# wenxuanliu/multimodal-vae

Measured on AMD Instinct MI355X. Metric: ELBO-steps/sec (whole node), MultiMNIST b=256 per GPU, higher is better.
Workload: dtype bf16; 1 GPU; multimnist_50x50_conv_mmvae_gru_text_3pass_elbo_step; batch_per_gpu=256, global_batch=256, n_latents=100, parallelism=dp1, hip_graph=False, optimizer=adam, mfma=bf16 in / fp32 acc; fp32 master weights, BN stats, PoE/KL/BCE/NLL, Adam

## Files before the change

### multimodal-vae_amd/csrc/gemm_small.hip

```cpp
#include "gemm.h"
#include <cstdlib>

namespace {

typedef __attribute__((ext_vector_type(4))) int i32x4;

__device__ __forceinline__ bf16x8 buf_load16(__amdgpu_buffer_rsrc_t rsrc, unsigned off) {
    const i32x4 v = __builtin_bit_cast(i32x4, __builtin_amdgcn_raw_buffer_load_b128(rsrc, (int)off, 0, 0));
    return __builtin_bit_cast(bf16x8, v);
}

__device__ __forceinline__ int fast_divmod(int r, int d, float inv, int& rem) {
    int q = (int)((float)r * inv);
    rem = r - q * d;
    if (rem < 0) { --q; rem += d; }
    else if (rem >= d) { ++q; rem -= d; }
    return q;
}

template <int MT, int NT, int KS, bool DGRAD>
__global__ __launch_bounds__(KS * 64) void gemm_small_kernel(const GemmParams p) {
    extern __shared__ __attribute__((aligned(16))) char smem[];
    const GatherCommon& c = p.c;
    const GatherClass& k = p.cls[blockIdx.z];
    const int tid = threadIdx.x, lane = tid & 63, wave = tid >> 6;
    const int fr = lane & 15, fq = lane >> 4;
    constexpr int RW = MT * 16, CW = NT * 16;
    const int tiles_per_group = (k.rows_per_group + RW - 1) / RW;
    if ((int)blockIdx.x >= tiles_per_group * c.groups) return;
    const int g = blockIdx.x / tiles_per_group;
    const int row0 = (blockIdx.x - g * tiles_per_group) * RW;
    const int n_base = blockIdx.y * CW;
    const int K = k.K, Kpad = k.Kpad;
    const int nch_all = (K + 63) / 64;
    const int ch0 = nch_all * wave / KS, ch1 = nch_all * (wave + 1) / KS;

    const int nimg_a = c.a_bcast_n > 0 ? c.a_bcast_n : c.groups * c.group_n;
    const __amdgpu_buffer_rsrc_t arsrc = __builtin_amdgcn_make_buffer_rsrc(
        const_cast<bf16*>(c.A), 0, (int)((size_t)nimg_a * c.AH * c.AW * c.Ald * sizeof(bf16)), 0x00020000);
    const __amdgpu_buffer_rsrc_t brsrc = __builtin_amdgcn_make_buffer_rsrc(
        const_cast<bf16*>(k.Wp), 0, (int)((size_t)p.npad * Kpad * sizeof(bf16)), 0x00020000);

    const int pix_per_img = k.OY * k.OX;
    const float inv_pix = 1.0f / (float)pix_per_img, inv_ox = 1.0f / (float)k.OX, inv_tw = 1.0f / (float)k.TW;
    int a_off[MT], opix[MT], dpix[MT], grow[MT];
    unsigned mtap[MT];
#pragma unroll
    for (int mt = 0; mt < MT; ++mt) {
        const int r = row0 + mt * 16 + fr;
        a_off[mt] = 0; mtap[mt] = 0; opix[mt] = -1; dpix[mt] = 0; grow[mt] = 0;
        if (r < k.rows_per_group) {
            int rem, ox;
            const int img = fast_divmod(r, pix_per_img, inv_pix, rem);
            const int oy = fast_divmod(rem, k.OX, inv_ox, ox);
            const int nimg = g * c.group_n + img;
            int aimg = nimg;
            if (c.a_bcast_n > 0) aimg %= c.a_bcast_n;
            const int y0 = oy * c.sy + k.offy, x0 = ox * c.sx + k.offx;
            a_off[mt] = (((aimg * c.AH + y0) * c.AW + x0) * c.Ald + fq * 8) * (int)sizeof(bf16);
            unsigned mx = 0, m = 0;
            for (int tx = 0; tx < k.TW; ++tx) mx |= ((unsigned)(x0 + tx * c.dx) < (unsigned)c.AW ? 1u : 0u) << tx;
            for (int ty = 0; ty < k.TH; ++ty)
                if ((unsigned)(y0 + ty * c.dy) < (unsigned)c.AH) m |= mx << (ty * k.TW);
            mtap[mt] = m;
            const int py = oy * c.osy + k.ooy, px = ox * c.osx + k.oox;
            opix[mt] = (nimg * c.OH + py) * c.OW + px;
            dpix[mt] = p.d_bcast_n > 0 ? ((nimg % p.d_bcast_n) * c.OH + py) * c.OW + px : opix[mt];
            grow[mt] = g * k.rows_per_group + r;
        }
    }
    const int ntaps = k.TH * k.TW;
    const int cshift = 31 - __clz(c.C);
    int b_off[NT];
#pragma unroll
// ... 135 lines not shown
                for (int j = 0; j < 4; ++j) {
                    float x = act_fwd(p.e_act, v[j]);
                    if (p.e_mask) x = ((mb >> (8 * j)) & 0xff) ? x * p.e_mask_scale : 0.f;
                    av[j] = x;
                }
            }
            const size_t o = (size_t)opix[mt] * p.ldo + n0;
            if (vec) {
                if (p.out_bf) {
                    bf16x4 ob;
#pragma unroll
                    for (int j = 0; j < 4; ++j) ob[j] = (bf16)v[j];
                    *reinterpret_cast<bf16x4*>(p.out_bf + o) = ob;
                }
                if (!DGRAD && p.out_act_bf) {
                    bf16x4 ob;
#pragma unroll
                    for (int j = 0; j < 4; ++j) ob[j] = (bf16)av[j];
                    *reinterpret_cast<bf16x4*>(p.out_act_bf + o) = ob;
                }
                if (p.out_f) *reinterpret_cast<f32x4*>(p.out_f + o) = f32x4{v[0], v[1], v[2], v[3]};
            } else {
                for (int j = 0; j < nv; ++j) {
                    if (p.out_bf) p.out_bf[o + j] = (bf16)v[j];
                    if (!DGRAD && p.out_act_bf) p.out_act_bf[o + j] = (bf16)av[j];
                    if (p.out_f) p.out_f[o + j] = v[j];
                }
            }
        }
        if (want_stats || want_red) {
            const int slot = (blockIdx.x + 5 * blockIdx.z) % MMVAE_STAT_SLOTS;
#pragma unroll
            for (int j = 0; j < 4; ++j) {
                float a = s1[j], b = s2[j];
#pragma unroll
                for (int o = 1; o < 16; o <<= 1) { a += __shfl_xor(a, o, 64); b += __shfl_xor(b, o, 64); }
                if (fr == 0 && j < nv) {
                    const int n = n0 + j;
                    float2* dst = want_stats ? p.colstats : p.d_red;
                    if (dst) {
                        const bool cm = !want_stats && p.d_cmod > 0;
                        const int tcol = cm ? n % p.d_cmod : n;
                        const int sl = (slot + (cm ? n / p.d_cmod : 0)) % MMVAE_STAT_SLOTS;
                        atomicAdd(&dst[(g * MMVAE_STAT_SLOTS + sl) * (cm ? p.d_cmod : c.N) + tcol].x, a);
                        atomicAdd(&dst[(g * MMVAE_STAT_SLOTS + sl) * (cm ? p.d_cmod : c.N) + tcol].y, b);
                    }
                    if (p.d_colsum) atomicAdd(p.d_colsum + n, a);
                }
            }
        }
    }
}

template <int MT, int NT, int KS, bool DGRAD>
int launch_small(const GemmParams& p, hipStream_t stream) {
    const GatherCommon& c = p.c;
    int max_tiles = 0;
    for (int i = 0; i < c.nclasses; ++i) max_tiles = max(max_tiles, ceil_div(p.cls[i].rows_per_group, MT * 16));
    dim3 grid(max_tiles * c.groups, ceil_div(c.N, NT * 16), c.nclasses);
    const size_t lds = KS > 1 ? (size_t)(KS - 1) * MT * NT * 4 * 64 * sizeof(float) : 0;
    if (mmvae_probe_on()) {
        char note[40];
        snprintf(note, sizeof(note), "small<%d,%d,%d,%s>", MT, NT, KS, DGRAD ? "dgrad" : "fwd");
        mmvae_probe_note(note);
    }
    MMVAE_LAUNCH((gemm_small_kernel<MT, NT, KS, DGRAD>), grid, dim3(KS * 64), lds, stream, p);
    return mmvae_check_launch("gemm_small");
}

template <int MT, int NT, bool DGRAD>
int launch_small_ks(const GemmParams& p, int ks, hipStream_t stream) {
    if (ks >= 4) return launch_small<MT, NT, 4, DGRAD>(p, stream);
    if (ks >= 2) return launch_small<MT, NT, 2, DGRAD>(p, stream);
    return launch_small<MT, NT, 1, DGRAD>(p, stream);
}

}

int try_launch_gemm_small(const GemmParams& pin, hipStream_t stream) {
    const GatherCommon& c = pin.c;
    int max_tiles128 = 0, min_nch = 1 << 30;
    long long tiles22 = 0, tiles44 = 0, rows_total = 0;
    for (int i = 0; i < c.nclasses; ++i) {
        const GatherClass& k = pin.cls[i];
        if (k.TH * k.TW > 1 && (c.C < 32 || (c.C & (c.C - 1)) != 0)) return 0;
        if (k.TH * k.TW > 32) return 0;
        max_tiles128 = max(max_tiles128, ceil_div(k.rows_per_group, 128));
        min_nch = min(min_nch, ceil_div(k.K, 64));
        tiles22 += (long long)ceil_div(k.rows_per_group, 32) * c.groups * ceil_div(c.N, 32);
        tiles44 += (long long)ceil_div(k.rows_per_group, 64) * c.groups * ceil_div(c.N, 64);
        rows_total += (long long)k.rows_per_group * c.groups;
    }
    const long long tiles128 = (long long)max_tiles128 * c.groups * c.nclasses * ceil_div(c.N, 128);
    if (tiles128 > 128) return 0;
    {
        constexpr double cap = 8.0;
        double fl = 0.0;
        for (int i = 0; i < c.nclasses; ++i) fl += 2.0 * pin.cls[i].rows_per_group * c.groups * c.N * pin.cls[i].K;
        if (cap > 0.0 && fl > cap * 1e9) return 0;
    }
    const long long nimg_a = c.a_bcast_n > 0 ? c.a_bcast_n : (long long)c.groups * c.group_n;
    if (nimg_a * c.AH * c.AW * c.Ald * 2 >= (1ll << 31)) return 0;
    if ((long long)c.groups * c.group_n * c.OH * c.OW >= (1ll << 31) || rows_total >= (1ll << 23)) return 0;
    GemmParams p = pin;
    p.ksplit = 1; p.sk_buf = nullptr;
    if (p.npad <= 0) p.npad = c.N <= 16 ? 16 : c.N <= 32 ? 32 : c.N <= 64 ? 64 : round_up(c.N, 128);
    (void)tiles44;
    if (tiles22 > 1536) return 0;
    if (p.d_r == nullptr && (p.d_mask || p.d_red || p.d_colsum)) return 0;
    constexpr long long wave_target = 1024;
    const int ks = (int)min((long long)min(4, max(1, min_nch / 2)), max(1ll, wave_target / max(tiles22, 1ll)));
    const int rc = p.d_r ? launch_small_ks<2, 2, true>(p, ks, stream) : launch_small_ks<2, 2, false>(p, ks, stream);
    return rc == MMVAE_OK ? 1 : rc;
}
```

### multimodal-vae_amd/csrc/multimnist.hip

```cpp
#include "multimnist.h"
#include <memory>
#include "mlp_tail.h"
#include "plan_base.h"
#include "thin.h"
#include "text_plan.h"
#include <cstring>

namespace {
constexpr int IMG = 50, NPIX = 2500;
}

struct MMPlan : PlanBase {
    int ldz, kx, kz;
    int lde;
    ConvL conv[4], convT[4];
    LinL fc[3], up;
    BnL bn[6];
    int H = TXT_H;
    const char *te_name = "text_encoder", *td_name = "text_decoder";
    TextGruIdx te_f, te_r, td0, td1;
    const float* step_image = nullptr;
    hipEvent_t ev_dz = nullptr;
    hipEvent_t ev_txtgrads = nullptr;
    int te_h2p, te_h2pT, g_te_h2p, td_z2h, td_z2hT, g_td_z2h, td_h2o, td_h2oT, g_td_h2o;
// ... 228 lines not shown
            g.c.A = r[l - 1]; g.tr = &tr;
            if (mmvae_knob("mm_stage_out", 1)) tr.out = a[l - 1];
        }
        MMVAE_TRY(launch_gemm_gather(g, s));
        const int rows = B * L.g.OH * L.g.OW;
        if (fuse && l <= 2) continue;
        MMVAE_TRY(bn_act(P, P.bn[L.bn], r[l], a[l], rows, rows, 1, w.st_e[l - 1], bn_updates, w.aff_e[l - 1], w.mr_e[l - 1], training, s));
    }
    {
        GatherPlan pl = plan_fwdform(2, 2, 1, 1, 256, 2, 2, 1, 0, 400, 1, rows);
        GemmParams g = gemm_of(P, pl, &P.fc[0].pk_fwd, 1, rows);
        g.c.A = w.a4; g.c.a_bcast_n = B;
        g.bias = P.buf.params + P.fc[0].b_off; g.out_bf = w.y1; g.ldo = 400;
        g.out_act_bf = w.ay1; g.e_act = ACT_SWISH; if (drop) { g.e_mask = m1; g.e_mask_scale = ms; }
        MMVAE_TRY(launch_gemm_gather(g, s));
    }
    }
    if (waist) {
        Mlp2Latent1FwdArgs a = *waist;
        a.rows = rows; a.x = w.ay1;
        a.w2 = P.buf.packed + P.pk.d[P.wa_w2].dst_off; a.b2 = P.buf.params + P.fc[1].b_off;
        a.w3 = P.buf.packed + P.pk.d[P.wa_w3].dst_off; a.b3 = P.buf.params + P.fc[2].b_off;
        if (drop) { a.mask = m2; a.mask_scale = ms; }
        a.y2 = w.y2; a.ay2 = w.ay2; a.out = out;
        return launch_mlp2_latent1_fwd(a, s);
    }
    if (P.mlp_tail) {
        Mlp2FwdArgs a{};
        a.rows = rows; a.x = w.ay1;
        a.w2 = P.buf.packed + P.pk.d[P.mt_w2].dst_off; a.b2 = P.buf.params + P.fc[1].b_off;
        a.w3 = P.buf.packed + P.pk.d[P.mt_w3].dst_off; a.b3 = P.buf.params + P.fc[2].b_off;
        if (drop) { a.mask = m2; a.mask_scale = ms; }
        a.y2 = w.y2; a.ay2 = w.ay2; a.out = out;
        return launch_mlp2_fwd(a, s);
    }
    {
        GatherPlan pl = dense_plan(rows, 400, 400, 200);
        GemmParams g = gemm_of(P, pl, &P.fc[1].pk_fwd, 1, rows);
        g.c.A = w.ay1;
        g.bias = P.buf.params + P.fc[1].b_off; g.out_bf = w.y2; g.ldo = 200;
        g.out_act_bf = w.ay2; g.e_act = ACT_SWISH; if (drop) { g.e_mask = m2; g.e_mask_scale = ms; }
        MMVAE_TRY(launch_gemm_gather(g, s));
    }
    {
        GatherPlan pl = dense_plan(rows, 200, 200, 2 * P.D);
        GemmParams g = gemm_of(P, pl, &P.fc[2].pk_fwd, 1, rows);
        g.c.A = w.ay2;
        g.bias = P.buf.params + P.fc[2].b_off; g.out_f = out; g.ldo = 2 * P.D;
        MMVAE_TRY(launch_gemm_gather(g, s));
    }
    return MMVAE_OK;
}

int enc_bwd(MMPlan& P, const bf16* d_out, int variants, const uint8_t* m1, const uint8_t* m2, int dropout, hipStream_t s, bool fuse = false,
            const Mlp2Latent1BwdArgs* waist = nullptr, float* loss_out = nullptr, bool tail_only = false) {
    MMPlan::W& w = P.w;
    const int B = P.B, rows = variants * B, D2 = 2 * P.D;
    const float ms = 1.f / (1.f - DROP_P);
    auto cls_w = std::make_shared<std::vector<WgradParams>>();
    if (waist) {
        Mlp2Latent1BwdArgs a = *waist;
        a.rows = rows;
        a.w3t = P.buf.packed + P.pk.d[P.wa_w3t].dst_off; a.w2t = P.buf.packed + P.pk.d[P.wa_w2t].dst_off;
        a.y2 = w.y2; a.y1 = w.y1;
        if (dropout) { a.mask2 = m2; a.mask1 = m1; a.mask_scale = ms; }
        a.dy2 = w.dy2; a.dy1 = w.dy1;
        a.db2 = P.buf.grads + P.fc[1].b_off; a.db1 = P.buf.grads + P.fc[0].b_off;
        a.d_enc_out = w.d_encout; a.lde = P.lde;
        MMVAE_TRY(launch_mlp2_latent1_bwd(a, s));
        {
            hipStream_t fs = s;
            MMVAE_TRY(wgrad_side_stream(P, s, &fs));
            MMVAE_TRY(launch_mlp2_latent1_finish(a.scratch, rows, P.D, P.buf.grads + P.fc[2].b_off, w.sums, loss_out, fs));
        }
        GatherPlan p3 = dense_plan(rows, 200, 200, D2);
        WgradParams g3 = wgrad_of(P, p3, &P.fc[2].gk, 1, rows);
        g3.c.A = w.ay2; g3.P = w.d_encout; g3.ldp = P.lde;
        MMVAE_TRY(wgrad_async(P, g3, s));
        GatherPlan p2 = dense_plan(rows, 400, 400, 200);
        WgradParams g2 = wgrad_of(P, p2, &P.fc[1].gk, 1, rows);
        g2.c.A = w.ay1; g2.P = w.dy2; g2.ldp = 200;
        MMVAE_TRY(wgrad_async(P, g2, s));
    } else if (P.mlp_tail) {
        {
            GatherPlan pl = dense_plan(rows, 200, 200, D2);
            WgradParams g = wgrad_of(P, pl, &P.fc[2].gk, 1, rows);
            g.c.A = w.ay2; g.P = d_out; g.ldp = P.lde;
            if (fuse) cls_w->push_back(g);
            else MMVAE_TRY(wgrad_async(P, g, s));
        }
        Mlp2BwdArgs a{};
        a.rows = rows; a.d_out = d_out;
        a.w3t = P.buf.packed + P.pk.d[P.mt_w3t].dst_off; a.w2t = P.buf.packed + P.pk.d[P.mt_w2t].dst_off;
        a.y2 = w.y2; a.y1 = w.y1;
        if (dropout) { a.mask2 = m2; a.mask1 = m1; a.mask_scale = ms; }
        a.dy2 = w.dy2; a.dy1 = w.dy1;
        a.db2 = P.buf.grads + P.fc[1].b_off; a.db1 = P.buf.grads + P.fc[0].b_off;
        MMVAE_TRY(launch_mlp2_bwd(a, s));
        GatherPlan pl = dense_plan(rows, 400, 400, 200);
        WgradParams g = wgrad_of(P, pl, &P.fc[1].gk, 1, rows);
        g.c.A = w.ay1; g.P = w.dy2; g.ldp = 200;
        if (fuse) cls_w->push_back(g);
        else MMVAE_TRY(wgrad_async(P, g, s));
    } else {
    {
        GatherPlan pl = dense_plan(rows, 200, 200, D2);
        WgradParams g = wgrad_of(P, pl, &P.fc[2].gk, 1, rows);
        g.c.A = w.ay2; g.P = d_out; g.ldp = P.lde;
        MMVAE_TRY(wgrad_async(P, g, s));
        GatherPlan pd = dense_plan(rows, P.lde, P.lde, 200);
        GemmParams d = gemm_of(P, pd, &P.fc[2].pk_dgrad, 1, rows);
        d.c.A = d_out; d.out_bf = w.dy2; d.ldo = 200;
        d.d_r = w.y2; d.d_ld = 200; d.d_act = ACT_SWISH; if (dropout) { d.d_mask = m2; d.d_mask_scale = ms; }
        d.d_colsum = P.buf.grads + P.fc[1].b_off;
        MMVAE_TRY(launch_gemm_gather(d, s));
    }
    {
        GatherPlan pl = dense_plan(rows, 400, 400, 200);
        WgradParams g = wgrad_of(P, pl, &P.fc[1].gk, 1, rows);
        g.c.A = w.ay1; g.P = w.dy2; g.ldp = 200;
        MMVAE_TRY(wgrad_async(P, g, s));
        GatherPlan pd = dense_plan(rows, 200, 200, 400);
        GemmParams d = gemm_of(P, pd, &P.fc[1].pk_dgrad, 1, rows);
        d.c.A = w.dy2; d.out_bf = w.dy1; d.ldo = 400;
        d.d_r = w.y1; d.d_ld = 400; d.d_act = ACT_SWISH; if (dropout) { d.d_mask = m1; d.d_mask_scale = ms; }
        d.d_colsum = P.buf.grads + P.fc[0].b_off;
        MMVAE_TRY(launch_gemm_gather(d, s));
    }
    }
    if (tail_only) return MMVAE_OK;
    {
        GatherPlan pl = plan_fwdform(2, 2, 1, 1, 256, 2, 2, 1, 0, 400, 1, rows);
        WgradParams g = wgrad_of(P, pl, &P.fc[0].gk, 1, rows);
        g.c.A = w.a4; g.c.a_bcast_n = B;
        g.P = w.dy1; g.ldp = 400;
        if (P.mlp_tail && fuse) {
            MMPlan* pp = &P;
            cls_w->push_back(g);
            side_later(P, [pp, cls_w](hipStream_t ws_) {
                MMVAE_TRY(launch_wgrad_group(cls_w->data(), (int)cls_w->size(), ws_, &pp->slab));
                return pp->batch_reduce ? MMVAE_OK : launch_wgrad_reduce(&pp->slab, ws_, true);
            }, mmvae_knob("mm_cls_lane", 1));
        } else {
            MMVAE_TRY(wgrad_async(P, g, s));
        }
        GatherPlan pd{};
        pd.c.AH = 1; pd.c.AW = 1; pd.c.Ald = 400; pd.c.C = 400; pd.c.sy = pd.c.sx = 1; pd.c.dy = pd.c.dx = 1;
        pd.c.OH = 2; pd.c.OW = 2; pd.c.osy = pd.c.osx = 1; pd.c.N = 256; pd.c.nclasses = 4;
        for (int sidx = 0; sidx < 4; ++sidx) {
            GatherClass& k = pd.cls[sidx];
            k.OY = 1; k.OX = 1; k.TH = 1; k.TW = 1; k.offy = 0; k.offx = 0; k.ooy = sidx / 2; k.oox = sidx % 2;
            k.K = 400; k.Kpad = round_up(400, 64);
        }
        GemmParams d = gemm_of(P, pd, P.fc[0].pk_dgrad4, 1, rows);
        d.c.A = w.dy1; d.out_bf = w.db4; d.ldo = 256;
        d.d_r = w.r4; d.d_ld = 256; d.d_bcast_n = B; d.d_act = ACT_SWISH;
        d.d_affine = w.aff_e[2]; d.d_meanrstd = w.mr_e[2]; d.d_red = w.red_e[2];
        MMVAE_TRY(launch_gemm_gather(d, s));
    }
    bf16* r[4] = {w.r1, w.r2, w.r3, w.r4};
    bf16* a[4] = {w.a1, w.a2, w.a3, w.a4};
    bf16* dr[4] = {w.d1e, w.d2e, w.d3e, w.dr4};
    bf16* drr[4] = {nullptr, w.d2er, w.d3er, nullptr};
    for (int l = 3; l >= 1; --l) {
        const ConvL& L = P.conv[l];
        const BnL& b = P.bn[L.bn];
        const int pix = L.g.OH * L.g.OW;
        const bool fl = fuse && l < 3;
        BnBwdApplyArgs x{};
        x.db = (l == 3) ? w.db4 : dr[l];
        x.db2 = (l == 3 && variants == 2) ? w.db4 + (size_t)B * 1024 : nullptr;
        x.r = r[l]; x.dr = fl ? drr[l] : dr[l]; x.rows = B * pix; x.C = L.g.Cout; x.ld = L.g.Cout; x.rows_per_group = B * pix; x.G = 1;
        x.red = w.red_e[l - 1]; x.meanrstd = w.mr_e[l - 1]; x.gamma = P.buf.params + b.w_off;
        x.dgamma = P.buf.grads + b.w_off; x.dbeta = P.buf.grads + b.b_off;
        if (!fl) MMVAE_TRY(launch_bn_bwd_apply(x, s));
        WgradParams gw = wgrad_of(P, L.fwd, L.gk, 1, B);
        gw.c.A = a[l - 1]; gw.P = x.dr; gw.ldp = L.g.Cout;
        if (fuse) {
            MMPlan* pp = &P;
            {
                const bool byp = mmvae_knob("mm_stage_out", 1) != 0;
                const bool actp = l >= 2 && !byp;
                const bool bnb = fl && !(byp && l == 2);
                const int prows = B * P.conv[l >= 2 ? l - 1 : 1].g.OH * P.conv[l >= 2 ? l - 1 : 1].g.OW;
                const BnL bp = P.bn[P.conv[l >= 2 ? l - 1 : 1].bn];
                const bf16* rin = r[l >= 2 ? l - 1 : 1]; bf16* ao = a[l >= 2 ? l - 1 : 1]; const float2* st = w.st_e[l >= 2 ? l - 2 : 0];
                WgradParams g0 = wgrad_of(P, L.fwd, L.gk, 1, B);
                g0.c.A = a[l - 1]; g0.P = x.dr; g0.ldp = L.g.Cout;
                side_later(P, [pp, x, g0, bnb, actp, bp, rin, ao, st, prows](hipStream_t ws_) {
                    if (bnb) MMVAE_TRY(launch_bn_bwd_apply(x, ws_));
                    if (actp) MMVAE_TRY(bn_act_side(*pp, bp, rin, ao, prows, prows, 1, st, 1, ws_));
                    return wgrad_on(*pp, g0, ws_);
                }, l == 1 ? 1 : l == 2 ? mmvae_knob("mm_conv3_lane", 0) : mmvae_knob("mm_conv4_lane", 0));
            }
            if (fuse && l == 1) MMVAE_TRY(side_flush(P, s));
        }
        {
            GemmParams d = gemm_of(P, L.dgrad, L.pk_dgrad, 1, B, L.pk_dgrad_f);
            d.c.A = dr[l]; d.out_bf = dr[l - 1]; d.ldo = L.g.Cin;
            d.d_r = r[l - 1]; d.d_ld = L.g.Cin; d.d_act = ACT_SWISH;
            if (l > 1) { d.d_affine = w.aff_e[l - 2]; d.d_meanrstd = w.mr_e[l - 2]; d.d_red = w.red_e[l - 2]; }
            GatherTransform tr{};
            if (fl) {
                tr.kind = 2; tr.r = r[l]; tr.red = w.red_e[l - 1]; tr.mr = w.mr_e[l - 1]; tr.gamma = P.buf.params + b.w_off;
                tr.inv_cnt = 1.f / (float)(B * pix); tr.groups = 1;
                if (l == 2 && mmvae_knob("mm_stage_out", 1)) {
                    tr.out = drr[l]; tr.dgamma = P.buf.grads + b.w_off; tr.dbeta = P.buf.grads + b.b_off;
                }
                d.tr = &tr;
            }
            const bool flush = fuse && P.wgrad_forked && (mmvae_knob("mm_forks", 0) ? l == 2 : l >= 2);
// ... 651 lines not shown
                hipStream_t s) {
    MMVAE_REQUIRE(P && z && image && loglik_x && words, "mmvae_mm_iw_score: null argument");
    MMVAE_TRY(iw_image_rows(P, ws, wsb, z, image, B, K, loglik_x, s, "mmvae_mm_iw_score"));
    TextDecArgs a = td_args(*P, z, 1, false);
    a.R = B * K; a.words = words;
    return launch_text_decoder_fwd(a, s);
}
int mm_iw_score_image(MMPlan* P, void* ws, size_t wsb, const float* z, const float* image, int B, int K, float* loglik_x, hipStream_t s) {
    MMVAE_REQUIRE(P && z && image && loglik_x, "mmvae_mm_iw_score_image: null argument");
    return iw_image_rows(P, ws, wsb, z, image, B, K, loglik_x, s, "mmvae_mm_iw_score_image");
}

static bool layer_gemm(MMPlan& P, const std::string& name, GemmParams& g) {
    MMPlan::W& w = P.w;
    const int B = P.B;
    bf16* r[4] = {w.r1, w.r2, w.r3, w.r4};
    bf16* a[4] = {w.a1, w.a2, w.a3, w.a4};
    bf16* dre[4] = {w.d1e, w.d2e, w.d3e, w.dr4};
    bf16* q[4] = {w.u, w.q1, w.q2, w.q3};
    bf16* aq[4] = {w.au, w.aq1, w.aq2, w.aq3};
    bf16* dq[4] = {w.du, w.d1, w.d2, w.d3};
    if (name == "enc_conv1") {
        GatherPlan pl = dense_plan(B * 625, 16, 16, 32);
        g = gemm_of(P, pl, P.conv[0].pk_fwd, 1, B * 625);
        g.c.A = w.patches1; g.out_bf = w.r1; g.ldo = 32; g.out_act_bf = w.a1; g.e_act = ACT_SWISH;
        return true;
    }
    for (int l = 1; l < 4; ++l) {
        const ConvL& L = P.conv[l];
        if (name == "enc_conv" + std::to_string(l + 1)) {
            g = gemm_of(P, L.fwd, L.pk_fwd, 1, B, L.pk_fwd_f);
            g.c.A = a[l - 1];
            g.out_bf = r[l]; g.ldo = L.g.Cout; g.colstats = w.st_e[l - 1];
            return true;
        }
        if (name == "enc_conv" + std::to_string(l + 1) + "_dgrad") {
            g = gemm_of(P, L.dgrad, L.pk_dgrad, 1, B, L.pk_dgrad_f);
            g.c.A = dre[l]; g.out_bf = dre[l - 1]; g.ldo = L.g.Cin;
            g.d_r = r[l - 1]; g.d_ld = L.g.Cin; g.d_act = ACT_SWISH;
            if (l > 1) { g.d_affine = w.aff_e[l - 2]; g.d_meanrstd = w.mr_e[l - 2]; g.d_red = w.red_e[l - 2]; }
            return true;
        }
    }
    {
        const int rows = 2 * B;
        const float ms = 1.f / (1.f - DROP_P);
        if (name == "enc_fc1") {
            GatherPlan pl = plan_fwdform(2, 2, 1, 1, 256, 2, 2, 1, 0, 400, 1, rows);
            g = gemm_of(P, pl, &P.fc[0].pk_fwd, 1, rows);
            g.c.A = w.a4; g.c.a_bcast_n = B; g.bias = P.buf.params + P.fc[0].b_off; g.out_bf = w.y1; g.ldo = 400;
            g.out_act_bf = w.ay1; g.e_act = ACT_SWISH; g.e_mask = w.m1; g.e_mask_scale = ms;
            return true;
        }
        if (name == "enc_fc2") {
            GatherPlan pl = dense_plan(rows, 400, 400, 200);
            g = gemm_of(P, pl, &P.fc[1].pk_fwd, 1, rows);
            g.c.A = w.ay1; g.bias = P.buf.params + P.fc[1].b_off; g.out_bf = w.y2; g.ldo = 200;
            g.out_act_bf = w.ay2; g.e_act = ACT_SWISH; g.e_mask = w.m2; g.e_mask_scale = ms;
            return true;
        }
        if (name == "enc_fc3") {
            GatherPlan pl = dense_plan(rows, 200, 200, 2 * P.D);
            g = gemm_of(P, pl, &P.fc[2].pk_fwd, 1, rows);
            g.c.A = w.ay2; g.bias = P.buf.params + P.fc[2].b_off; g.out_f = w.tmp_f32; g.ldo = 2 * P.D;
            return true;
        }
        if (name == "enc_fc3_dgrad") {
            GatherPlan pd = dense_plan(rows, P.lde, P.lde, 200);
            g = gemm_of(P, pd, &P.fc[2].pk_dgrad, 1, rows);
            g.c.A = w.d_encout; g.out_bf = w.dy2; g.ldo = 200;
            g.d_r = w.y2; g.d_ld = 200; g.d_act = ACT_SWISH; g.d_mask = w.m2; g.d_mask_scale = ms;
            g.d_colsum = w.tmp_f32;
            return true;
        }
        if (name == "enc_fc2_dgrad") {
            GatherPlan pd = dense_plan(rows, 200, 200, 400);
            g = gemm_of(P, pd, &P.fc[1].pk_dgrad, 1, rows);
            g.c.A = w.dy2; g.out_bf = w.dy1; g.ldo = 400;
            g.d_r = w.y1; g.d_ld = 400; g.d_act = ACT_SWISH; g.d_mask = w.m1; g.d_mask_scale = ms;
            g.d_colsum = w.tmp_f32;
            return true;
        }
        if (name == "dec_up") {
            GatherPlan pl = dense_plan(3 * B, P.ldz, P.ldz, 1024);
            g = gemm_of(P, pl, &P.up.pk_fwd, 1, 3 * B);
            g.c.A = w.z_bf; g.out_bf = w.u; g.ldo = 1024; g.out_act_bf = w.au; g.e_act = ACT_SWISH;
            return true;
        }
        if (name == "dec_up_dgrad") {
            GatherPlan pd = dense_plan(rows, 1024, 1024, P.D);
            g = gemm_of(P, pd, &P.up.pk_dgrad, 1, rows);
            g.c.A = w.du; g.out_f = w.tmp_f32; g.ldo = P.D;
            return true;
        }
    }
    if (name == "dec_last_dgrad_gemm") {
        const ConvL& L = P.convT[3];
        GatherPlan pl = dense_plan(B * 625, 16, 16, 32);
        g = gemm_of(P, pl, L.pk_dgrad, 2, B * 625);
        g.c.A = w.patches4; g.out_bf = w.d3; g.ldo = 32;
        g.d_r = w.q3; g.d_ld = 32; g.d_act = ACT_SWISH; g.d_affine = w.aff_d[2]; g.d_meanrstd = w.mr_d[2]; g.d_red = w.red_d[2];
        return true;
    }
    for (int l = 0; l < 3; ++l) {
        const ConvL& L = P.convT[l];
        if (name == "dec_convT" + std::to_string(l + 1)) {
// ... 197 lines not shown
```

Before: 1828 ELBO-steps/s.

## Add register-prefetch pipelined small GEMM kernel with flattened scalar args

Measured after the change: 1848 ELBO-steps/s (median of 6 runs). +1.0%, better.

```diff
diff --git a/multimodal-vae_amd/csrc/gemm_small.hip b/multimodal-vae_amd/csrc/gemm_small.hip
--- a/multimodal-vae_amd/csrc/gemm_small.hip
+++ b/multimodal-vae_amd/csrc/gemm_small.hip
@@ -19,7 +19,7 @@
 }
 
 template <int MT, int NT, int KS, bool DGRAD>
-__global__ __launch_bounds__(KS * 64) void gemm_small_kernel(const GemmParams p) {
+__global__ __launch_bounds__(KS * 64) void gemm_small_kernel_v0(const GemmParams p) {
     extern __shared__ __attribute__((aligned(16))) char smem[];
     const GatherCommon& c = p.c;
     const GatherClass& k = p.cls[blockIdx.z];
@@ -261,6 +261,363 @@
     }
 }
 
+struct SmallCls {
+    int OY, OX, rows_per_group, TH, TW, offy, offx, ooy, oox, K, Kpad, w_bytes;
+    const bf16* Wp;
+};
+enum { SM_AFFINE = 1, SM_MASK = 2, SM_OUT_BF = 4, SM_OUT_F = 8, SM_OUT_ACT = 16, SM_STATS = 32, SM_COLSUM = 64, SM_CMOD = 128 };
+struct SmallArgs {
+    const bf16* A; const bf16* d_r;
+    const float* bias; const float2* d_affine; const float2* d_meanrstd; const uint8_t* mask;
+    bf16* out_bf; float* out_f; bf16* out_act_bf;
+    float2* stats;
+    float* d_colsum;
+    int a_bytes, bias_bytes, aff_bytes, mr_bytes, mask_bytes;
+    int groups, group_n, a_bcast_n, d_bcast_n;
+    int AH, AW, Ald, C, sy, sx, dy, dx;
+    int OH, OW, osy, osx, N, ldo, d_ld;
+    int cmod;
+    float inv_cmod;
+    int act;
+    float mask_scale;
+    unsigned flags;
+    SmallCls cls[MMVAE_MAX_CLASSES];
+};
+
+__device__ __forceinline__ float buf_load_f32(__amdgpu_buffer_rsrc_t rsrc, unsigned off) {
+    return __builtin_bit_cast(float, __builtin_amdgcn_raw_buffer_load_b32(rsrc, (int)off, 0, 0));
+}
+__device__ __forceinline__ float2 buf_load_f32x2(__amdgpu_buffer_rsrc_t rsrc, unsigned off) {
+    return __builtin_bit_cast(float2, __builtin_amdgcn_raw_buffer_load_b64(rsrc, (int)off, 0, 0));
+}
+
+template <int MT, int NT, int KS, bool DGRAD, bool VEC, int DEPTH>
+__global__ __launch_bounds__(KS * 64) void gemm_small_kernel(const SmallArgs a) {
+    extern __shared__ __attribute__((aligned(16))) char smem[];
+    const SmallCls k = a.cls[blockIdx.z];
+    asm volatile("" ::"s"(a.A), "s"(a.d_r), "s"(a.bias), "s"(a.d_affine), "s"(a.d_meanrstd), "s"(a.mask), "s"(a.out_bf), "s"(a.out_f),
+                 "s"(a.out_act_bf), "s"(a.stats), "s"(a.d_colsum), "s"(k.Wp), "s"(a.a_bytes), "s"(a.bias_bytes), "s"(a.aff_bytes),
+                 "s"(a.mr_bytes), "s"(a.mask_bytes), "s"(a.groups), "s"(a.group_n), "s"(a.a_bcast_n), "s"(a.d_bcast_n), "s"(a.AH),
+                 "s"(a.AW), "s"(a.Ald), "s"(a.C), "s"(a.sy), "s"(a.sx), "s"(a.dy), "s"(a.dx));
+    asm volatile("" ::"s"(a.OH), "s"(a.OW), "s"(a.osy), "s"(a.osx), "s"(a.N), "s"(a.ldo), "s"(a.d_ld), "s"(a.cmod), "s"(a.inv_cmod),
+                 "s"(a.act), "s"(a.mask_scale), "s"(a.flags), "s"(k.OY), "s"(k.OX), "s"(k.rows_per_group), "s"(k.TH), "s"(k.TW),
+                 "s"(k.offy), "s"(k.offx), "s"(k.ooy), "s"(k.oox), "s"(k.K), "s"(k.Kpad), "s"(k.w_bytes));
+    const int tid = threadIdx.x, lane = tid & 63;
+    const int wave = __builtin_amdgcn_readfirstlane(tid >> 6);
+    const int fr = lane & 15, fq = lane >> 4;
+    constexpr int RW = MT * 16, CW = NT * 16;
+    const int tiles_per_group = (k.rows_per_group + RW - 1) / RW;
+    if ((int)blockIdx.x >= tiles_per_group * a.groups) return;
+    const int g = blockIdx.x / tiles_per_group;
+    const int row0 = (blockIdx.x - g * tiles_per_group) * RW;
+    const int n_base = blockIdx.y * CW;
+    const int K = k.K, Kpad = k.Kpad, N = a.N;
+    const int nch_all = (K + 63) / 64;
+    const int ch0 = nch_all * wave / KS, ch1 = nch_all * (wave + 1) / KS;
+    const int nch = ch1 - ch0;
+    const unsigned flags = a.flags;
+
+    const __amdgpu_buffer_rsrc_t arsrc = __builtin_amdgcn_make_buffer_rsrc(const_cast<bf16*>(a.A), 0, a.a_bytes, 0x00020000);
+    const __amdgpu_buffer_rsrc_t brsrc = __builtin_amdgcn_make_buffer_rsrc(const_cast<bf16*>(k.Wp), 0, k.w_bytes, 0x00020000);
+
+    const int pix_per_img = k.OY * k.OX;
+    const float inv_pix = 1.0f / (float)pix_per_img, inv_ox = 1.0f / (float)k.OX, inv_tw = 1.0f / (float)k.TW;
+    int a_off[MT], opix[MT], dpix[MT], grow[MT];
+    unsigned mtap[MT];
+#pragma unroll
+    for (int mt = 0; mt < MT; ++mt) {
+        const int r = row0 + mt * 16 + fr;
+        a_off[mt] = 0; mtap[mt] = 0; opix[mt] = -1; dpix[mt] = 0; grow[mt] = 0;
+        if (r < k.rows_per_group) {
+            int rem, ox;
+            const int img = fast_divmod(r, pix_per_img, inv_pix, rem);
+            const int oy = fast_divmod(rem, k.OX, inv_ox, ox);
+            const int nimg = g * a.group_n + img;
+            int aimg = nimg;
+            if (a.a_bcast_n > 0) aimg %= a.a_bcast_n;
+            const int y0 = oy * a.sy + k.offy, x0 = ox * a.sx + k.offx;
+            a_off[mt] = (((aimg * a.AH + y0) * a.AW + x0) * a.Ald + fq * 8) * (int)sizeof(bf16);
+            unsigned mx = 0, m = 0;
+            for (int tx = 0; tx < k.TW; ++tx) mx |= ((unsigned)(x0 + tx * a.dx) < (unsigned)a.AW ? 1u : 0u) << tx;
+            for (int ty = 0; ty < k.TH; ++ty)
+                if ((unsigned)(y0 + ty * a.dy) < (unsigned)a.AH) m |= mx << (ty * k.TW);
+            mtap[mt] = m;
+            const int py = oy * a.osy + k.ooy, px = ox * a.osx + k.oox;
+            opix[mt] = (nimg * a.OH + py) * a.OW + px;
+            dpix[mt] = a.d_bcast_n > 0 ? ((nimg % a.d_bcast_n) * a.OH + py) * a.OW + px : opix[mt];
+            grow[mt] = g * k.rows_per_group + r;
+        }
+    }
+
+    float bias4[NT][4];
+    float2 aff[NT][4], mrs[NT][4];
+    int tcol[NT][4], tdiv[NT][4];
+    unsigned rbits[MT][NT][VEC ? 2 : 4];
+    unsigned mb[MT][NT];
+    if (KS == 1 || wave == 0) {
+        const __amdgpu_buffer_rsrc_t bias_rsrc = __builtin_amdgcn_make_buffer_rsrc(const_cast<float*>(a.bias), 0, a.bias_bytes, 0x00020000);
+        const __amdgpu_buffer_rsrc_t aff_rsrc = __builtin_amdgcn_make_buffer_rsrc(const_cast<float2*>(a.d_affine), 0, a.aff_bytes, 0x00020000);
+        const __amdgpu_buffer_rsrc_t mr_rsrc = __builtin_amdgcn_make_buffer_rsrc(const_cast<float2*>(a.d_meanrstd), 0, a.mr_bytes, 0x00020000);
+        const __amdgpu_buffer_rsrc_t mask_rsrc = __builtin_amdgcn_make_buffer_rsrc(const_cast<uint8_t*>(a.mask), 0, a.mask_bytes, 0x00020000);
+#pragma unroll
+        for (int nt = 0; nt < NT; ++nt) {
+            const int n0 = n_base + nt * 16 + fq * 4;
+#pragma unroll
+            for (int j = 0; j < 4; ++j) {
+                const int n = min(n0 + j, N - 1);
+                tcol[nt][j] = n; tdiv[nt][j] = 0;
+                if (flags & SM_CMOD) { int rem; tdiv[nt][j] = fast_divmod(n, a.cmod, a.inv_cmod, rem); tcol[nt][j] = rem; }
+            }
+#pragma unroll
+            for (int j = 0; j < 4; ++j) {
+                bias4[nt][j] = buf_load_f32(bias_rsrc, (unsigned)min(n0 + j, N - 1) * 4u);
+                if (DGRAD) {
+                    aff[nt][j] = buf_load_f32x2(aff_rsrc, (unsigned)(g * a.cmod + tcol[nt][j]) * 8u);
+                    mrs[nt][j] = buf_load_f32x2(mr_rsrc, (unsigned)(g * a.cmod + tcol[nt][j]) * 8u);
+                }
+            }
+#pragma unroll
+            for (int mt = 0; mt < MT; ++mt) {
+                if (DGRAD) {
+                    if (VEC) {
+                        const uint2 rv = *reinterpret_cast<const uint2*>(a.d_r + (size_t)dpix[mt] * a.d_ld + min(n0, N - 4));
+                        rbits[mt][nt][0] = rv.x; rbits[mt][nt][1] = rv.y;
+                    } else {
+                        const unsigned short* rp = reinterpret_cast<const unsigned short*>(a.d_r) + (size_t)dpix[mt] * a.d_ld;
+#pragma unroll
+                        for (int j = 0; j < 4; ++j) rbits[mt][nt][j] = rp[min(n0 + j, N - 1)];
+                    }
+                }
+                const unsigned moff = (unsigned)(grow[mt] * N + n0);
+                if (VEC) {
+                    mb[mt][nt] = __builtin_amdgcn_raw_buffer_load_b32(mask_rsrc, (int)moff, 0, 0);
+                } else {
+                    unsigned m = 0;
+#pragma unroll
+                    for (int j = 0; j < 4; ++j)
+                        m |= (unsigned)(__builtin_amdgcn_raw_buffer_load_b8(mask_rsrc, (int)(moff + j), 0, 0) ? 1 : 0) << (8 * j);
+                    mb[mt][nt] = m;
+                }
+            }
+        }
+    }
+
+    const int ntaps = k.TH * k.TW;
+    const int cshift = 31 - __clz(a.C);
+    int b_off[NT];
+#pragma unroll
+    for (int nt = 0; nt < NT; ++nt) b_off[nt] = ((n_base + nt * 16 + fr) * Kpad + fq * 8) * (int)sizeof(bf16);
+
+    auto load_chunk = [&](int ch, bf16x8 (&fa)[2][MT], bf16x8 (&fb)[2][NT]) {
+        const bool live = ch < ch1;
+#pragma unroll
+        for (int ks = 0; ks < 2; ++ks) {
+            const int kk0 = ch * 64 + ks * 32;
+            int tap = 0, acb = kk0;
+            if (ntaps > 1) { tap = kk0 >> cshift; acb = kk0 & (a.C - 1); }
+            const int ty = (int)(((float)tap + 0.5f) * inv_tw), tx = tap - ty * k.TW;
+            const int toff = (((ty * a.dy) * a.AW + tx * a.dx) * a.Ald + acb) * (int)sizeof(bf16);
+            const bool kin = live & (kk0 + fq * 8 < K);
+#pragma unroll
+            for (int mt = 0; mt < MT; ++mt) {
+                const unsigned bit = (mtap[mt] >> (tap & 31)) & (unsigned)kin;
+                fa[ks][mt] = buf_load16(arsrc, (unsigned)(a_off[mt] + toff) | (bit - 1u));
+            }
+#pragma unroll
+            for (int nt = 0; nt < NT; ++nt)
+                fb[ks][nt] = buf_load16(brsrc, (live & (kk0 < Kpad)) ? (unsigned)(b_off[nt] + kk0 * (int)sizeof(bf16)) : 0xFFFFFFFFu);
+        }
+    };
+    f32x4 acc[MT][NT];
+#pragma unroll
+    for (int mt = 0; mt < MT; ++mt)
+#pragma unroll
+        for (int nt = 0; nt < NT; ++nt) acc[mt][nt] = f32x4{0.f, 0.f, 0.f, 0.f};
+    auto compute_chunk = [&](bf16x8 (&fa)[2][MT], bf16x8 (&fb)[2][NT]) {
+#pragma unroll
+        for (int ks = 0; ks < 2; ++ks)
+#pragma unroll
+            for (int mt = 0; mt < MT; ++mt)
+#pragma unroll
+                for (int nt = 0; nt < NT; ++nt)
+                    acc[mt][nt] = __builtin_amdgcn_mfma_f32_16x16x32_bf16(fb[ks][nt], fa[ks][mt], acc[mt][nt], 0, 0, 0);
+    };
+
+    bf16x8 ra[DEPTH][2][MT], rb[DEPTH][2][NT];
+#pragma unroll
+    for (int i = 0; i < DEPTH; ++i) load_chunk(ch0 + i, ra[i], rb[i]);
+#pragma unroll 1
+    for (int base = 0; base < nch; base += DEPTH) {
+#pragma unroll
+        for (int i = 0; i < DEPTH; ++i) {
+            if (base + i < nch) compute_chunk(ra[i], rb[i]);
+            __builtin_amdgcn_sched_barrier(0);
+            if (nch > DEPTH) load_chunk(ch0 + base + i + DEPTH, ra[i], rb[i]);
+            __builtin_amdgcn_sched_barrier(0);
+        }
+    }
+
+    if (KS > 1) {
+        float* red = reinterpret_cast<float*>(smem);
+        if (wave > 0) {
+#pragma unroll
+            for (int mt = 0; mt < MT; ++mt)
+#pragma unroll
+                for (int nt = 0; nt < NT; ++nt)
+#pragma unroll
+                    for (int j = 0; j < 4; ++j)
+                        red[((wave - 1) * (MT * NT * 4) + (mt * NT + nt) * 4 + j) * 64 + lane] = acc[mt][nt][j];
+        }
+        __syncthreads();
+        if (wave > 0) return;
+#pragma unroll
+        for (int w = 0; w < KS - 1; ++w)
+#pragma unroll
+            for (int mt = 0; mt < MT; ++mt)
+#pragma unroll
+                for (int nt = 0; nt < NT; ++nt)
+#pragma unroll
+                    for (int j = 0; j < 4; ++j)
+                        acc[mt][nt][j] += red[(w * (MT * NT * 4) + (mt * NT + nt) * 4 + j) * 64 + lane];
+    }
+
+    const bool has_mask = (flags & SM_MASK) != 0;
+    const bool want_stats = !DGRAD && (flags & SM_STATS) != 0;
+    const bool want_red = DGRAD && (flags & (SM_STATS | SM_COLSUM)) != 0;
+#pragma unroll
+    for (int nt = 0; nt < NT; ++nt) {
+        const int n0 = n_base + nt * 16 + fq * 4;
+        if (n0 >= N) continue;
+        const int nv = VEC ? 4 : min(4, N - n0);
+        float dsc[4], dsh[4], dmean[4], drstd[4], s1[4], s2[4];
+#pragma unroll
+        for (int j = 0; j < 4; ++j) {
+            dsc[j] = (flags & SM_AFFINE) ? aff[nt][j].x : 1.f; dsh[j] = (flags & SM_AFFINE) ? aff[nt][j].y : 0.f;
+            dmean[j] = mrs[nt][j].x; drstd[j] = mrs[nt][j].y; s1[j] = 0.f; s2[j] = 0.f;
+        }
+#pragma unroll
+        for (int mt = 0; mt < MT; ++mt) {
+            if (opix[mt] < 0) continue;
+            float v[4];
+#pragma unroll
+            for (int j = 0; j < 4; ++j) v[j] = acc[mt][nt][j] + bias4[nt][j];
+            const unsigned mbits = mb[mt][nt];
+            if (DGRAD) {
+                float rr[4];
+#pragma unroll
+                for (int j = 0; j < 4; ++j) {
+                    const unsigned b = VEC ? ((j & 1) ? rbits[mt][nt][j >> 1] & 0xffff0000u : rbits[mt][nt][j >> 1] << 16) : rbits[mt][nt][VEC ? 0 : j] << 16;
+                    rr[j] = j < nv ? __builtin_bit_cast(float, b) : 0.f;
+                }
+#pragma unroll
+                for (int j = 0; j < 4; ++j) {
+                    float x = v[j] * act_bwd(a.act, rr[j] * dsc[j] + dsh[j]);
+                    if (has_mask) x = ((mbits >> (8 * j)) & 0xff) ? x * a.mask_scale : 0.f;
+                    v[j] = x;
+                    if (want_red && j < nv) { s1[j] += x; s2[j] += x * (rr[j] - dmean[j]) * drstd[j]; }
+                }
+            }
+            if (want_stats) {
+#pragma unroll
+                for (int j = 0; j < 4; ++j)
+                    if (j < nv) { s1[j] += v[j]; s2[j] += v[j] * v[j]; }
+            }
+            float av[4];
+            if (!DGRAD && (flags & SM_OUT_ACT)) {
+#pragma unroll
+                for (int j = 0; j < 4; ++j) {
+                    float x = act_fwd(a.act, v[j]);
+                    if (has_mask) x = ((mbits >> (8 * j)) & 0xff) ? x * a.mask_scale : 0.f;
+                    av[j] = x;
+                }
+            }
+            const size_t o = (size_t)opix[mt] * a.ldo + n0;
+            if (VEC) {
+                if (flags & SM_OUT_BF) {
+                    bf16x4 ob;
+#pragma unroll
+                    for (int j = 0; j < 4; ++j) ob[j] = (bf16)v[j];
+                    *reinterpret_cast<bf16x4*>(a.out_bf + o) = ob;
+                }
+                if (!DGRAD && (flags & SM_OUT_ACT)) {
+                    bf16x4 ob;
+#pragma unroll
+                    for (int j = 0; j < 4; ++j) ob[j] = (bf16)av[j];
+                    *reinterpret_cast<bf16x4*>(a.out_act_bf + o) = ob;
+                }
+                if (flags & SM_OUT_F) *reinterpret_cast<f32x4*>(a.out_f + o) = f32x4{v[0], v[1], v[2], v[3]};
+            } else {
+                for (int j = 0; j < nv; ++j) {
+                    if (flags & SM_OUT_BF) a.out_bf[o + j] = (bf16)v[j];
+                    if (!DGRAD && (flags & SM_OUT_ACT)) a.out_act_bf[o + j] = (bf16)av[j];
+                    if (flags & SM_OUT_F) a.out_f[o + j] = v[j];
+                }
+            }
+        }
+        if (want_stats || want_red) {
+            const int slot = (blockIdx.x + 5 * blockIdx.z) % MMVAE_STAT_SLOTS;
+#pragma unroll
+            for (int j = 0; j < 4; ++j) {
+                float sa = s1[j], sb = s2[j];
+#pragma unroll
+                for (int o = 1; o < 16; o <<= 1) { sa += __shfl_xor(sa, o, 64); sb += __shfl_xor(sb, o, 64); }
+                if (fr == 0 && j < nv) {
+                    const int n = n0 + j;
+                    if (flags & SM_STATS) {
+                        const int sl = (slot + tdiv[nt][j]) % MMVAE_STAT_SLOTS;
+                        atomicAdd(&a.stats[(g * MMVAE_STAT_SLOTS + sl) * a.cmod + tcol[nt][j]].x, sa);
+                        atomicAdd(&a.stats[(g * MMVAE_STAT_SLOTS + sl) * a.cmod + tcol[nt][j]].y, sb);
+                    }
+                    if (DGRAD && (flags & SM_COLSUM)) atomicAdd(a.d_colsum + n, sa);
+                }
+            }
+        }
+    }
+}
+
+template <bool DGRAD>
+SmallArgs flatten_small(const GemmParams& p) {
+    const GatherCommon& c = p.c;
+    SmallArgs a{};
+    const long long nimg_a = c.a_bcast_n > 0 ? c.a_bcast_n : (long long)c.groups * c.group_n;
+    a.A = c.A; a.a_bytes = (int)((size_t)nimg_a * c.AH * c.AW * c.Ald * sizeof(bf16));
+    a.groups = c.groups; a.group_n = c.group_n; a.a_bcast_n = c.a_bcast_n; a.d_bcast_n = p.d_bcast_n;
+    a.AH = c.AH; a.AW = c.AW; a.Ald = c.Ald; a.C = c.C; a.sy = c.sy; a.sx = c.sx; a.dy = c.dy; a.dx = c.dx;
+    a.OH = c.OH; a.OW = c.OW; a.osy = c.osy; a.osx = c.osx; a.N = c.N; a.ldo = p.ldo; a.d_ld = p.d_ld;
+    int rows_max = 0;
+    for (int i = 0; i < c.nclasses; ++i) {
+        const GatherClass& k = p.cls[i];
+        SmallCls& s = a.cls[i];
+        s.OY = k.OY; s.OX = k.OX; s.rows_per_group = k.rows_per_group; s.TH = k.TH; s.TW = k.TW; s.offy = k.offy; s.offx = k.offx;
+        s.ooy = k.ooy; s.oox = k.oox; s.K = k.K; s.Kpad = k.Kpad; s.w_bytes = (int)((size_t)p.npad * k.Kpad * sizeof(bf16)); s.Wp = k.Wp;
+        rows_max = max(rows_max, k.rows_per_group);
+    }
+    const bool cm = DGRAD && p.d_cmod > 0;
+    a.cmod = cm ? p.d_cmod : c.N; a.inv_cmod = 1.0f / (float)a.cmod;
+    const void* none = c.A;
+    a.bias = p.bias ? p.bias : (const float*)none; a.bias_bytes = p.bias ? c.N * (int)sizeof(float) : 0;
+    const bool aff = DGRAD && p.d_affine, mr = DGRAD && p.d_meanrstd;
+    const int tab_bytes = c.groups * a.cmod * (int)sizeof(float2);
+    a.d_affine = aff ? p.d_affine : (const float2*)none; a.aff_bytes = aff ? tab_bytes : 0;
+    a.d_meanrstd = mr ? p.d_meanrstd : (const float2*)none; a.mr_bytes = mr ? tab_bytes : 0;
+    const uint8_t* mask = DGRAD ? p.d_mask : (p.out_act_bf ? p.e_mask : nullptr);
+    a.mask = mask ? mask : (const uint8_t*)none; a.mask_bytes = mask ? c.groups * rows_max * c.N : 0;
+    a.mask_scale = DGRAD ? p.d_mask_scale : p.e_mask_scale;
+    a.act = DGRAD ? p.d_act : p.e_act;
+    a.d_r = p.d_r; a.out_bf = p.out_bf; a.out_f = p.out_f; a.out_act_bf = DGRAD ? nullptr : p.out_act_bf;
+    a.stats = DGRAD ? p.d_red : p.colstats; a.d_colsum = DGRAD ? p.d_colsum : nullptr;
+    a.flags = (aff ? SM_AFFINE : 0) | (mask ? SM_MASK : 0) | (a.out_bf ? SM_OUT_BF : 0) | (a.out_f ? SM_OUT_F : 0) |
+              (a.out_act_bf ? SM_OUT_ACT : 0) | (a.stats ? SM_STATS : 0) | (a.d_colsum ? SM_COLSUM : 0) | (cm ? SM_CMOD : 0);
+    return a;
+}
+
+template <int MT, int NT, int KS, bool DGRAD, bool VEC>
+void launch_small_depth(const SmallArgs& a, int depth, dim3 grid, size_t lds, hipStream_t stream) {
+    if (depth == 2) MMVAE_LAUNCH((gemm_small_kernel<MT, NT, KS, DGRAD, VEC, 2>), grid, dim3(KS * 64), lds, stream, a);
+    else if (depth == 3) MMVAE_LAUNCH((gemm_small_kernel<MT, NT, KS, DGRAD, VEC, 3>), grid, dim3(KS * 64), lds, stream, a);
+    else MMVAE_LAUNCH((gemm_small_kernel<MT, NT, KS, DGRAD, VEC, 4>), grid, dim3(KS * 64), lds, stream, a);
+}
+
 template <int MT, int NT, int KS, bool DGRAD>
 int launch_small(const GemmParams& p, hipStream_t stream) {
     const GatherCommon& c = p.c;
@@ -273,7 +630,15 @@
         snprintf(note, sizeof(note), "small<%d,%d,%d,%s>", MT, NT, KS, DGRAD ? "dgrad" : "fwd");
         mmvae_probe_note(note);
     }
-    MMVAE_LAUNCH((gemm_small_kernel<MT, NT, KS, DGRAD>), grid, dim3(KS * 64), lds, stream, p);
+    const int depth = mmvae_knob("gemm_small_prefetch", 2);
+    if (depth <= 0) {
+        MMVAE_LAUNCH((gemm_small_kernel_v0<MT, NT, KS, DGRAD>), grid, dim3(KS * 64), lds, stream, p);
+    } else {
+        const SmallArgs a = flatten_small<DGRAD>(p);
+        const bool vec = c.N % 4 == 0 && p.ldo % 4 == 0 && (!DGRAD || p.d_ld % 4 == 0);
+        if (vec) launch_small_depth<MT, NT, KS, DGRAD, true>(a, depth, grid, lds, stream);
+        else launch_small_depth<MT, NT, KS, DGRAD, false>(a, depth, grid, lds, stream);
+    }
     return mmvae_check_launch("gemm_small");
 }
 
diff --git a/multimodal-vae_amd/csrc/multimnist.hip b/multimodal-vae_amd/csrc/multimnist.hip
--- a/multimodal-vae_amd/csrc/multimnist.hip
+++ b/multimodal-vae_amd/csrc/multimnist.hip
@@ -304,6 +304,23 @@
     return MMVAE_OK;
 }
 
+static GemmParams fc1_dgrad_gemm(MMPlan& P, int rows) {
+    MMPlan::W& w = P.w;
+    GatherPlan pd{};
+    pd.c.AH = 1; pd.c.AW = 1; pd.c.Ald = 400; pd.c.C = 400; pd.c.sy = pd.c.sx = 1; pd.c.dy = pd.c.dx = 1;
+    pd.c.OH = 2; pd.c.OW = 2; pd.c.osy = pd.c.osx = 1; pd.c.N = 256; pd.c.nclasses = 4;
+    for (int sidx = 0; sidx < 4; ++sidx) {
+        GatherClass& k = pd.cls[sidx];
+        k.OY = 1; k.OX = 1; k.TH = 1; k.TW = 1; k.offy = 0; k.offx = 0; k.ooy = sidx / 2; k.oox = sidx % 2;
+        k.K = 400; k.Kpad = round_up(400, 64);
+    }
+    GemmParams d = gemm_of(P, pd, P.fc[0].pk_dgrad4, 1, rows);
+    d.c.A = w.dy1; d.out_bf = w.db4; d.ldo = 256;
+    d.d_r = w.r4; d.d_ld = 256; d.d_bcast_n = P.B; d.d_act = ACT_SWISH;
+    d.d_affine = w.aff_e[2]; d.d_meanrstd = w.mr_e[2]; d.d_red = w.red_e[2];
+    return d;
+}
+
 int enc_bwd(MMPlan& P, const bf16* d_out, int variants, const uint8_t* m1, const uint8_t* m2, int dropout, hipStream_t s, bool fuse = false,
             const Mlp2Latent1BwdArgs* waist = nullptr, float* loss_out = nullptr, bool tail_only = false) {
     MMPlan::W& w = P.w;
@@ -396,19 +413,7 @@
         } else {
             MMVAE_TRY(wgrad_async(P, g, s));
         }
-        GatherPlan pd{};
-        pd.c.AH = 1; pd.c.AW = 1; pd.c.Ald = 400; pd.c.C = 400; pd.c.sy = pd.c.sx = 1; pd.c.dy = pd.c.dx = 1;
-        pd.c.OH = 2; pd.c.OW = 2; pd.c.osy = pd.c.osx = 1; pd.c.N = 256; pd.c.nclasses = 4;
-        for (int sidx = 0; sidx < 4; ++sidx) {
-            GatherClass& k = pd.cls[sidx];
-            k.OY = 1; k.OX = 1; k.TH = 1; k.TW = 1; k.offy = 0; k.offx = 0; k.ooy = sidx / 2; k.oox = sidx % 2;
-            k.K = 400; k.Kpad = round_up(400, 64);
-        }
-        GemmParams d = gemm_of(P, pd, P.fc[0].pk_dgrad4, 1, rows);
-        d.c.A = w.dy1; d.out_bf = w.db4; d.ldo = 256;
-        d.d_r = w.r4; d.d_ld = 256; d.d_bcast_n = B; d.d_act = ACT_SWISH;
-        d.d_affine = w.aff_e[2]; d.d_meanrstd = w.mr_e[2]; d.d_red = w.red_e[2];
-        MMVAE_TRY(launch_gemm_gather(d, s));
+        MMVAE_TRY(launch_gemm_gather(fc1_dgrad_gemm(P, rows), s));
     }
     bf16* r[4] = {w.r1, w.r2, w.r3, w.r4};
     bf16* a[4] = {w.a1, w.a2, w.a3, w.a4};
@@ -1166,6 +1171,7 @@
             g.out_act_bf = w.ay1; g.e_act = ACT_SWISH; g.e_mask = w.m1; g.e_mask_scale = ms;
             return true;
         }
+        if (name == "enc_fc1_dgrad") { g = fc1_dgrad_gemm(P, rows); return true; }
         if (name == "enc_fc2") {
             GatherPlan pl = dense_plan(rows, 400, 400, 200);
             g = gemm_of(P, pl, &P.fc[1].pk_fwd, 1, rows);
```
